# tudelft/CUAHN-VIO

Hardware: AMD Instinct MI355X
Metric: homography preds/sec (frame pairs/s), full 4-block HomographyNet @ 320x224 (higher is better)
Workload: dtype f32 as 2 x fp16 planes (three fp16 MFMAs per product, fp32 accumulate)

## Files before the change

cuahn_vio_amd/csrc/capi_weights.hip:

```cpp
#include "capi_internal.h"

using namespace hnet;

namespace capi {

bool parse_blob(const uint8_t* p, size_t len, Blob& out) {
    if (len < 12 || memcmp(p, "HNETW001", 8) != 0) return false;
    uint32_t n; memcpy(&n, p + 8, 4);
    if (n > 1024) return false;
    size_t pos = 12;
    struct Ent { std::string name; std::vector<uint32_t> dims; uint64_t off; size_t count; };
    std::vector<Ent> ents;
    for (uint32_t i = 0; i < n; i++) {
        if (pos + 4 > len) return false;
        uint32_t ln; memcpy(&ln, p + pos, 4); pos += 4;
        if (ln > 512 || pos + ln + 4 > len) return false;
        Ent e; e.name.assign((const char*)p + pos, ln); pos += ln;
        uint32_t nd; memcpy(&nd, p + pos, 4); pos += 4;
        if (nd > 8 || pos + 4 * nd + 8 > len) return false;
        e.count = 1;
        for (uint32_t d = 0; d < nd; d++) {
            uint32_t v; memcpy(&v, p + pos, 4); pos += 4;
            e.dims.push_back(v);
            if (v != 0 && e.count > (len / 4) / v) return false;
            e.count *= v;
        }
        memcpy(&e.off, p + pos, 8); pos += 8;
        if (e.off % 4) return false;
        ents.push_back(e);
    }
    const size_t data0 = (pos + 63) / 64 * 64;
    if (data0 > len) return false;
    const size_t room = len - data0;
    for (auto& e : ents) {
        if (e.off > room || e.count > (room - (size_t)e.off) / 4) return false;
        out.t.push_back({e.name, Tensor{e.dims, (const float*)(p + data0 + e.off), e.count}});
    }
    return true;
}

template <typename T>
static hipError_t upload(T** dst, const std::vector<T>& v) {
    hipError_t e = dalloc(dst, v.size());
    if (e != hipSuccess) return e;
    return hipMemcpy(*dst, v.data(), v.size() * sizeof(T), hipMemcpyHostToDevice);
}

static std::vector<float> pack_conv(const float* w, const ConvDesc& d, int kp) {
    const int rl = d.ks * d.cin, rlp = kp / d.ks;
    std::vector<float> out((size_t)d.cout * kp, 0.0f);
    for (int co = 0; co < d.cout; co++)
        for (int ci = 0; ci < d.cin; ci++)
            for (int kh = 0; kh < d.ks; kh++)
                for (int kw = 0; kw < d.ks; kw++) {
                    const int r = kw * d.cin + ci;
                    (void)rl;
                    out[(size_t)co * kp + kh * rlp + r] = w[(((size_t)co * d.cin + ci) * d.ks + kh) * d.ks + kw];
                }
    return out;
}

static std::vector<float> pack_first_weights(const float* w, int cout) {
    const int nfrag = cout == 8 ? 28 : 56;
    std::vector<float> out((size_t)nfrag * 64, 0.0f);
    for (int t = 0; t < nfrag; t++)
        for (int l = 0; l < 64; l++) {
            int kh, kk, n;
            if (cout == 8) { kh = t / 4; kk = 4 * (l >> 4) + (t % 4); n = l & 15; }
            else { kh = t / 8; const int q = (t % 8) / 4, e = t % 4; kk = 8 * q + 4 * (l >> 5) + e; n = l & 31; }
            const int kwp = kk >> 1, ci = kk & 1, dx = n / cout, co = n % cout, kw = kwp - dx;
            if (kw >= 0 && kw < 7) out[(size_t)t * 64 + l] = w[(((size_t)co * 2 + ci) * 7 + kh) * 7 + kw];
        }
    return out;
}

static std::vector<float> permute_fc(const float* w, int n_out) {
    std::vector<float> out((size_t)n_out * 5120);
    for (int o = 0; o < n_out; o++)
        for (int c = 0; c < 256; c++)
            for (int pix = 0; pix < 20; pix++) out[(size_t)o * 5120 + pix * 256 + c] = w[(size_t)o * 5120 + c * 20 + pix];
    return out;
}

static inline void wsplit_gemm(float w, int np, uint16_t& a, uint16_t& b, uint16_t& c3) {
    if (np == 2) { split2h(w, a, b); c3 = 0; }
    else split3(w, a, b, c3);
}
int upload_weights(hnet_ctx* c, const Blob& b) {
#define CK(expr)                                                                    \
    do {                                                                            \
        hipError_t e_ = (expr);                                                     \
        if (e_ != hipSuccess) {                                                     \
            fprintf(stderr, "hnet weights: %s: %s\n", #expr, hipGetErrorString(e_)); \
            return HNET_ERR_DEVICE;                                                 \
        }                                                                           \
    } while (0)
    {
        auto fr = [](auto*& p) { if (p) (void)hipFree(p); p = nullptr; };
        for (int l = 0; l < 20; l++) { fr(c->patch_frag[l]); fr(c->conv_w[l]); fr(c->conv_b[l]); fr(c->conv_w16[l]); fr(c->conv_wfrag[l]); fr(c->chain_w[l]); }
        for (int k = 0; k < 3; k++) { fr(c->fc_w[k]); fr(c->fc_b[k]); }
        fr(c->s2_frag[0]); fr(c->s2_frag[3]); fr(c->b30_frag); fr(c->b40_frag); fr(c->b41_frag); fr(c->w1_16); fr(c->b3f_w1); fr(c->b42_w2); fr(c->b42_w3);
        fr(c->w1); fr(c->b1); fr(c->w2); fr(c->b2);
    }
    for (int l = 0; l < 20; l++) {
        const ConvDesc& d = kConvs[l];
        const std::string pre = std::string(d.block == 4 ? "model_last_block_list.0." : "model_part1.") + d.name + ".0.";
        const Tensor* w = b.find(pre + "weight", {(uint32_t)d.cout, (uint32_t)d.cin, (uint32_t)d.ks, (uint32_t)d.ks});
        const Tensor* bi = b.find(pre + "bias", {(uint32_t)d.cout});
        if (!w || !bi) return HNET_ERR_BAD_WEIGHTS;
        if (c->s3 && c->n_planes == 2 && chain_layer(l)) {
            std::vector<uint16_t> fr;
            if (!chain_pack_weights(l, w->data, fr)) return HNET_ERR_BAD_WEIGHTS;
            CK(upload(&c->chain_w[l], fr));
        }
        if (c->s3 && l == 13) {
            std::vector<uint16_t> fr((size_t)5 * 3 * 64 * 8, 0);
            for (int ln = 0; ln < 64; ln++) {
                const int n = ln & 15, gg = ln >> 4, dx = n >> 3, co = n & 7;
                for (int e = 0; e < 4; e++) {
                    const int kk = 4 * gg + e, kw = (kk >> 1) - dx, ci = kk & 1;
                    if (kw < 0 || kw >= 7) continue;
                    uint16_t sp[3];
                    wsplit_np(w->data[(((size_t)co * 2 + ci) * 7 + 6) * 7 + kw], c->n_planes, sp[0], sp[1], sp[2]);
                    for (int pl = 0; pl < 3; pl++) fr[(((size_t)4 * 3 + pl) * 64 + ln) * 8 + e] = sp[pl];
                }
            }
            for (int st = 0; st < 4; st++)
                for (int ln = 0; ln < 64; ln++) {
                    const int n = ln & 15, gg = ln >> 4, kh = 2 * st + (gg >> 1);
                    if (kh >= 7) continue;
                    const int dx = n >> 3, co = n & 7;
                    for (int j = 0; j < 8; j++) {
                        const int kk = 8 * (gg & 1) + j, kw = (kk >> 1) - dx, ci = kk & 1;
                        if (kw < 0 || kw >= 7) continue;
                        uint16_t sp[3];
                        wsplit_np(w->data[(((size_t)co * 2 + ci) * 7 + kh) * 7 + kw], c->n_planes, sp[0], sp[1], sp[2]);
                        for (int pl = 0; pl < 3; pl++) fr[(((size_t)st * 3 + pl) * 64 + ln) * 8 + j] = sp[pl];
                    }
                }
            CK(upload(&c->b40_frag, fr));
        }
        if (c->s3 && l == 7) {
            std::vector<uint16_t> fr((size_t)7 * 3 * 64 * 8, 0);
            for (int kh = 0; kh < 7; kh++)
                for (int ln = 0; ln < 64; ln++) {
                    const int n = ln & 31, hh = ln >> 5, dx = n >> 4, co = n & 15;
                    for (int j = 0; j < 8; j++) {
                        const int kk = 8 * hh + j, kw = (kk >> 1) - dx, ci = kk & 1;
                        if (kw < 0 || kw >= 7) continue;
                        uint16_t sp[3];
                        wsplit_np(w->data[(((size_t)co * 2 + ci) * 7 + kh) * 7 + kw], c->n_planes, sp[0], sp[1], sp[2]);
                        for (int pl = 0; pl < 3; pl++) fr[(((size_t)kh * 3 + pl) * 64 + ln) * 8 + j] = sp[pl];
                    }
                }
            CK(upload(&c->b30_frag, fr));
            c->b30_s3 = true;
        }
        if (c->s3 && l == 8 && c->n_planes == 2) {
            std::vector<uint16_t> f2((size_t)2 * 13 * 2 * 64 * 8, 0);
            for (int nt = 0; nt < 2; nt++)
                for (int st = 0; st < 13; st++)
                    for (int ln = 0; ln < 64; ln++) {
                        const int co = 16 * nt + (ln & 15), gg = ln >> 4, t = 2 * st + (gg >> 1);
                        if (t >= 25) continue;
                        const int kh = t / 5, kw = t % 5;
                        for (int j = 0; j < 8; j++) {
                            const int ci = 8 * (gg & 1) + j;
                            uint16_t a0, a1;
                            split2h(w->data[(((size_t)co * 16 + ci) * 5 + kh) * 5 + kw], a0, a1);
                            f2[((((size_t)nt * 13 + st) * 2 + 0) * 64 + ln) * 8 + j] = a0;
                            f2[((((size_t)nt * 13 + st) * 2 + 1) * 64 + ln) * 8 + j] = a1;
                        }
                    }
            CK(upload(&c->b3f_w1, f2));
        }
        if (c->s3 && (l == 15 || l == 16) && c->n_planes == 2) {
            const int nnt = d.cout / 16, nst = l == 15 ? 5 : 9;
            std::vector<uint16_t> f2((size_t)nnt * nst * 2 * 64 * 8, 0);
            for (int nt = 0; nt < nnt; nt++)
                for (int st = 0; st < nst; st++)
                    for (int ln = 0; ln < 64; ln++) {
                        const int co = 16 * nt + (ln & 15), gg = ln >> 4;
                        const int t = l == 15 ? 2 * st + (gg >> 1) : st;
                        if (t >= 9) continue;
                        const int kh = t / 3, kw = t % 3;
                        for (int j = 0; j < 8; j++) {
                            const int ci = l == 15 ? 8 * (gg & 1) + j : 8 * gg + j;
                            uint16_t a0, a1;
                            split2h(w->data[(((size_t)co * d.cin + ci) * 3 + kh) * 3 + kw], a0, a1);
                            f2[((((size_t)nt * nst + st) * 2 + 0) * 64 + ln) * 8 + j] = a0;
                            f2[((((size_t)nt * nst + st) * 2 + 1) * 64 + ln) * 8 + j] = a1;
                        }
                    }
            CK(upload(l == 15 ? &c->b42_w2 : &c->b42_w3, f2));
        }
        if (c->s3 && conv_is_first_s2(l)) {
            const int nt_n = d.cout / 16;
            std::vector<uint16_t> fr((size_t)nt_n * 4 * 3 * 64 * 8, 0);
            for (int nt = 0; nt < nt_n; nt++)
                for (int st = 0; st < 4; st++)
                    for (int ln = 0; ln < 64; ln++) {
                        const int co = nt * 16 + (ln & 15), gg = ln >> 4, kh = 2 * st + (gg >> 1);
                        if (kh >= 7) continue;
                        for (int j = 0; j < 8; j++) {
                            const int kw = 4 * (gg & 1) + (j >> 1), ci = j & 1;
                            if (kw >= 7) continue;
                            uint16_t sp[3];
                            wsplit_np(w->data[(((size_t)co * 2 + ci) * 7 + kh) * 7 + kw], c->n_planes, sp[0], sp[1], sp[2]);
                            for (int pl = 0; pl < 3; pl++) fr[((((size_t)nt * 4 + st) * 3 + pl) * 64 + ln) * 8 + j] = sp[pl];
                        }
                    }
            CK(upload(&c->s2_frag[l], fr));
            c->first_s2 = true;
        }
        if (c->s3 && conv_is_patch32_layer(l)) {
            std::vector<uint16_t> fr((size_t)4 * 9 * 3 * 64 * 8, 0);
            for (int nt = 0; nt < 4; nt++)
                for (int st = 0; st < 9; st++)
                    for (int ln = 0; ln < 64; ln++) {
                        const int n = nt * 16 + (ln & 15), gg = ln >> 4, kh = st / 3, kw = st % 3;
                        for (int j = 0; j < 8; j++) {
                            const int ci = 8 * gg + j;
                            uint16_t sp[3];
                            wsplit_np(w->data[(((size_t)n * 32 + ci) * 3 + kh) * 3 + kw], c->n_planes, sp[0], sp[1], sp[2]);
                            for (int pl = 0; pl < 3; pl++) fr[((((size_t)nt * 9 + st) * 3 + pl) * 64 + ln) * 8 + j] = sp[pl];
                        }
                    }
            CK(upload(&c->patch_frag[l], fr));
        }
        if (c->s3 && conv_is_patch_layer(l)) {
            const int ks = d.ks, nstep = (ks * ks + 1) / 2;
            std::vector<uint16_t> fr((size_t)2 * nstep * 3 * 64 * 8, 0);
            for (int nt = 0; nt < 2; nt++)
                for (int st = 0; st < nstep; st++)
                    for (int ln = 0; ln < 64; ln++) {
                        const int n = nt * 16 + (ln & 15), gg = ln >> 4, t = 2 * st + (gg >> 1);
                        if (t >= ks * ks) continue;
                        const int kh = t / ks, kw = t % ks;
                        for (int j = 0; j < 8; j++) {
                            const int ci = 8 * (gg & 1) + (((gg & 1) && !c->patch_b128) ? (j + 4) % 8 : j);
                            uint16_t sp[3];
                            wsplit_np(w->data[(((size_t)n * 16 + ci) * ks + kh) * ks + kw], c->n_planes, sp[0], sp[1], sp[2]);
                            for (int pl = 0; pl < 3; pl++) fr[((((size_t)nt * nstep + st) * 3 + pl) * 64 + ln) * 8 + j] = sp[pl];
                        }
                    }
            CK(upload(&c->patch_frag[l], fr));
        }
        if (conv_is_first_direct(l)) CK(upload(&c->conv_w[l], pack_first_weights(w->data, d.cout)));
        else {
            const std::vector<float> packed = pack_conv(w->data, d, conv_padded_k(l));
            CK(upload(&c->conv_w[l], packed));
            if (c->s3 && l == 14) {
                std::vector<uint16_t> fr((size_t)7 * 3 * 64 * 8, 0);
                for (int st = 0; st < 7; st++)
                    for (int ln = 0; ln < 64; ln++) {
                        const int n = ln & 15, gg = ln >> 4, t = c->n_planes == 2 ? b41_tap(st, gg) : 4 * st + gg;
                        if (t < 0 || t >= 25) continue;
                        const int kh = t / 5, kw = t % 5;
                        for (int j = 0; j < 8; j++) {
                            const int ci = (c->n_planes != 2 && (gg & 1)) ? (j + 4) % 8 : j;
                            uint16_t sp[3];
                            wsplit_np(w->data[(((size_t)n * 8 + ci) * 5 + kh) * 5 + kw], c->n_planes, sp[0], sp[1], sp[2]);
                            for (int pl = 0; pl < 3; pl++) fr[(((size_t)st * 3 + pl) * 64 + ln) * 8 + j] = sp[pl];
                        }
                    }
                CK(upload(&c->b41_frag, fr));
            }
            if (c->s3 && conv_is_s3_layer(l)) {
                std::vector<uint16_t> pl(packed.size() * 3);
                for (size_t i = 0; i < packed.size(); i++)
                    wsplit_gemm(packed[i], c->n_planes, pl[i], pl[packed.size() + i], pl[2 * packed.size() + i]);
                CK(upload(&c->conv_w16[l], pl));
            }
            if (c->n_planes == 2 && conv_region_layer(l)) {
                const int ntap = d.ks * d.ks, ntap_pad = conv_region_taps_padded(l), nchunk = d.cin / 64;
                std::vector<uint16_t> fr((size_t)(d.cout / 16) * nchunk * ntap_pad * 2 * 2 * 64 * 8, 0);
                for (int nt = 0; nt < d.cout / 16; nt++)
                    for (int cc = 0; cc < nchunk; cc++)
                        for (int t = 0; t < ntap; t++)
                            for (int st = 0; st < 2; st++)
                                for (int ln = 0; ln < 64; ln++)
                                    for (int e = 0; e < 8; e++) {
                                        const int n = nt * 16 + (ln & 15), ci = 64 * cc + 32 * st + 8 * (ln >> 4) + e;
                                        uint16_t sp[3];
                                        wsplit_gemm(w->data[(((size_t)n * d.cin + ci) * d.ks + t / d.ks) * d.ks + t % d.ks], 2, sp[0], sp[1], sp[2]);
                                        const size_t base = ((((size_t)(nt * nchunk + cc) * ntap_pad + t) * 2 + st) * 2) * 64 * 8;
                                        fr[base + (size_t)ln * 8 + e] = sp[0];
                                        fr[base + 64 * 8 + (size_t)ln * 8 + e] = sp[1];
                                    }
                CK(upload(&c->conv_wfrag[l], fr));
            }
        }
        CK(upload(&c->conv_b[l], std::vector<float>(bi->data, bi->data + d.cout)));
    }
    for (int k = 0; k < 3; k++) {
        const std::string pre = "model_part1.fc_block_" + std::to_string(k + 1) + ".";
        const Tensor* w = b.find(pre + "weight", {8, 5120});
        const Tensor* bi = b.find(pre + "bias", {8});
        if (!w || !bi) return HNET_ERR_BAD_WEIGHTS;
        CK(upload(&c->fc_w[k], permute_fc(w->data, 8)));
        CK(upload(&c->fc_b[k], std::vector<float>(bi->data, bi->data + 8)));
    }
    {
        static const char* heads[2] = {"fc_block_4_mean", "fc_block_4_uncertainty"};
        std::vector<float> w1, b1, w2, b2;
        for (int h = 0; h < 2; h++) {
            const std::string pre = std::string("model_last_block_list.0.") + heads[h] + ".";
            const Tensor* tw1 = b.find(pre + "1.weight", {256, 5120});
            const Tensor* tb1 = b.find(pre + "1.bias", {256});
            const Tensor* tw2 = b.find(pre + "4.weight", {8, 256});
            const Tensor* tb2 = b.find(pre + "4.bias", {8});
            if (!tw1 || !tb1 || !tw2 || !tb2) return HNET_ERR_BAD_WEIGHTS;
            std::vector<float> p = permute_fc(tw1->data, 256);
            w1.insert(w1.end(), p.begin(), p.end());
            b1.insert(b1.end(), tb1->data, tb1->data + 256);
            w2.insert(w2.end(), tw2->data, tw2->data + 8 * 256);
            b2.insert(b2.end(), tb2->data, tb2->data + 8);
        }
        CK(upload(&c->w1, w1)); CK(upload(&c->b1, b1)); CK(upload(&c->w2, w2)); CK(upload(&c->b2, b2));
        c->w1_feat_scale = 1.0f;
        if (c->s3) {
            int e = 0;
            if (c->n_planes == 2) {
                float m = 0.f;
                for (float v : w1) m = std::max(m, std::fabs(v));
                if (m > 0.f && m < 0x1p-15f) e = std::min(-7 - std::ilogb(m), 24);
            }
            const float up = std::ldexp(1.0f, e);
            c->w1_feat_scale = std::ldexp(1.0f, -e);
            std::vector<uint16_t> pl(w1.size() * 3);
            for (size_t i = 0; i < w1.size(); i++) wsplit_gemm(w1[i] * up, c->n_planes, pl[i], pl[w1.size() + i], pl[2 * w1.size() + i]);
            CK(upload(&c->w1_16, pl));
        }
    }

    return HNET_OK;
#undef CK
}

}
```

cuahn_vio_amd/csrc/igemm_region.h:

```cpp
#pragma once
#include "igemm_pipe.h"

namespace hnet {

template <int CIN_, int KS_, int P_, int RP_, bool KSPLIT_, int HI_, int WI_>
struct RegionCfg {
    static constexpr int CIN = CIN_, KS = KS_, P = P_, RP = RP_, PAD = (KS_ - 1) / 2;
    static constexpr int HI = HI_, WI = WI_, HO = (HI_ + 1) / 2, WO = WI_ / 2;
    static_assert(WI_ % 2 == 0, "the parity images assume an even input width");
    static constexpr bool KSPLIT = KSPLIT_;
    static constexpr int TM = 5, BM = 80, BN = KSPLIT_ ? 64 : 128, NWAVE = 8, NT = 512;
    static constexpr int NCHUNK = CIN / 64, NTAP = KS * KS;
    static constexpr int TAPS_X = KSPLIT_ ? (NTAP + 1) / 2 : NTAP;
    static constexpr int NTAP_PAD = KSPLIT_ ? 2 * TAPS_X : NTAP;
    static constexpr int DEPTH = 5;
    static_assert((2 * TAPS_X) % DEPTH == 0, "weight-fragment ring");
    static constexpr int REG_PLANE = (RP + 16) * 64;
    static constexpr int REG_BUF = 2 * REG_PLANE;
    static constexpr int LDS_BYTES = 2 * REG_BUF * 2;
    static constexpr int RG = RP / 8;
    static_assert(RP % 8 == 0 && LDS_BYTES <= 160 * 1024 && CIN % 64 == 0, "region");
    static constexpr size_t wfrag_halves(int n) { return (size_t)(n / 16) * NCHUNK * NTAP_PAD * 2 * 2 * 64 * 8; }
};

template <class C, bool OUT32>
__global__ __launch_bounds__(512, 2) void igemm_s3_region_kernel(S3Params p) {
    constexpr int TM = C::TM, BN = C::BN, NWAVE = C::NWAVE, CIN = C::CIN, KS = C::KS, PAD = C::PAD;
    constexpr int REG_PLANE = C::REG_PLANE, REG_BUF = C::REG_BUF, NTAP = C::NTAP, NCHUNK = C::NCHUNK;
    constexpr int DEPTH = C::DEPTH, NTAP_PAD = C::NTAP_PAD;
    extern __shared__ __attribute__((aligned(16))) uint16_t smem_r[];

    const int tid = threadIdx.x, lane = tid & 63;
    const int wave = __builtin_amdgcn_readfirstlane(tid >> 6);
    const int khalf = C::KSPLIT ? wave >> 2 : 0, wn = C::KSPLIT ? wave & 3 : wave;
    constexpr int R = C::HO * C::WO, HW = C::HI * C::WI;
    const int rows_tile = C::P * R;
    int mt, n0;
    {
        const int nx = gridDim.x, ny = gridDim.y, total = nx * ny;
        const int lin = blockIdx.x + blockIdx.y * nx;
        const int xcd = lin & 7, idx = lin >> 3;
        const int base = total >> 3, rem = total & 7;
        const int Lt = xcd * base + min(xcd, rem) + idx;
        mt = Lt / ny;
        n0 = (Lt % ny) * BN;
    }
    const int m0 = mt * rows_tile, pair0 = mt * C::P;
    const int m_end = min(p.M, m0 + rows_tile);
    const int px_total = (p.M / R) * HW;

    const __amdgpu_buffer_rsrc_t rA = __builtin_amdgcn_make_buffer_rsrc((void*)p.A, 0, 0x7FFFFFF0, 0x00020000);
    const __amdgpu_buffer_rsrc_t rW = __builtin_amdgcn_make_buffer_rsrc((void*)p.Wp, 0, 0x7FFFFFF0, 0x00020000);
    const int a_pl = (int)(p.a_plane * 2);

    {
        const u32x4 z = {0u, 0u, 0u, 0u};
        *reinterpret_cast<u32x4*>(&smem_r[(tid >> 8) * REG_BUF + ((tid >> 7) & 1) * REG_PLANE + C::RP * 64 + (tid & 127) * 8]) = z;
    }

    const int grow = lane >> 3, gphys = lane & 7;
    constexpr int RGW = (C::RG + NWAVE - 1) / NWAVE;
    constexpr int Wo = C::WO, hh_e = (C::HI + 1) >> 1, hh_o = C::HI >> 1;
    constexpr int ps_e = (hh_e * Wo + 1) & ~1, ps_o = (hh_o * Wo + 1) & ~1;
    constexpr int base2 = 2 * C::P * ps_e;
    uint32_t rvoff[RGW];
#pragma unroll
    for (int j = 0; j < RGW; j++) {
        const int q = (wave + NWAVE * j) * 8 + grow;
        const int yo = q >= base2, qq = yo ? q - base2 : q, ps = yo ? ps_o : ps_e, hh = yo ? hh_o : hh_e;
        const int xo = qq >= C::P * ps, q3 = xo ? qq - C::P * ps : qq;
        const int pl_ = yo ? q3 / ps_o : q3 / ps_e;
        const int t = q3 - pl_ * ps, Y = t / Wo, xh = t - Y * Wo;
        const int T = pl_ * R + t;
        const int gq = (pair0 + pl_) * HW + (2 * Y + yo) * C::WI + 2 * xh + xo;
        const bool ok = q < base2 + 2 * C::P * ps_o && t < hh * Wo && gq < px_total;
        rvoff[j] = ok ? (uint32_t)((gq * CIN + (gphys ^ (2 * ((T >> 1) & 3))) * 8) * 2) : S3_OOB;
    }
    auto dma_region = [&](int c) {
#pragma unroll
        for (int j = 0; j < RGW; j++) {
            const int g = wave + NWAVE * j;
            if (g < C::RG) {
                const uint32_t vo = rvoff[j];
#pragma unroll
                for (int pl = 0; pl < 2; pl++) {
                    const int so = c * 128 + pl * a_pl;
                    __builtin_amdgcn_raw_ptr_buffer_load_lds(rA, (lds_ptr_t)(smem_r + (c & 1) * REG_BUF + pl * REG_PLANE + g * 512), 16, vo, so, 0, 0);
                }
            }
        }
    };

    const uint32_t wlane = (uint32_t)(lane * 16);
    const int wtile0 = ((n0 >> 4) + wn) * (NCHUNK * NTAP_PAD);
    const int t_lo_w = khalf * C::TAPS_X;
    bf16x8 fw[DEPTH][2];
    auto load_w = [&](int slot, int c, int sidx) {
#if defined(HNET_REGION_ABLATE) && HNET_REGION_ABLATE == 1
        if (c | (sidx >= DEPTH)) return;
#endif
        const int so = (wtile0 + c * NTAP_PAD + t_lo_w) * 4096 + sidx * 2048;
#pragma unroll
        for (int pl = 0; pl < 2; pl++) {
            const int so2 = so + pl * 1024;
            fw[slot][pl] = __builtin_bit_cast(bf16x8, __builtin_amdgcn_raw_buffer_load_b128(rW, wlane, so2, 0));
        }
    };

    const int r16 = lane & 15, g16 = lane >> 4;
    int qe_b[TM], qo_b[TM], tt0[TM];
    uint32_t okb[TM];
#pragma unroll
    for (int i = 0; i < TM; i++) {
        const int ml = i * 16 + r16;
        const bool ok = m0 + ml < m_end;
        const int pl_ = ml / R, rem = ml - pl_ * R, oy = rem / Wo, ox = rem - oy * Wo;
        const int t0 = oy * Wo + ox;
        qe_b[i] = (pl_ * ps_e + t0) * 128;
        qo_b[i] = (base2 + pl_ * ps_o + t0) * 128;
        tt0[i] = pl_ * R + t0;
        uint32_t bits = 0;
#pragma unroll
        for (int k = 0; k < KS; k++) {
            bits |= ((unsigned)(2 * oy - PAD + k) < (unsigned)C::HI) ? (1u << k) : 0u;
            bits |= ((unsigned)(2 * ox - PAD + k) < (unsigned)C::WI) ? (1u << (8 + k)) : 0u;
        }
        okb[i] = ok ? bits : 0u;
    }
    bf16x8 fa[2][TM][2];
    int a_byte[TM];
    constexpr int xoff_e = C::P * ps_e * 128, xoff_o = C::P * ps_o * 128;
    auto tap_addr = [&](int t) {
#if defined(HNET_REGION_ABLATE) && HNET_REGION_ABLATE == 2
        if (t != t_lo_w) return;
#endif
        const int kh = t / KS, kw = t - kh * KS;
        const int ey = kh - PAD, ex = kw - PAD;
        const int yo = ey & 1, xo = ex & 1, dt = (ey >> 1) * Wo + (ex >> 1);
        const int s_b = (xo ? (yo ? xoff_o : xoff_e) : 0) + dt * 128;
        const uint32_t need = t < NTAP ? ((1u << kh) | (1u << (8 + kw))) : 0xFFFFFFFFu;
#pragma unroll
        for (int i = 0; i < TM; i++) {
            int t0_ = tt0[i], qs_ = yo ? qo_b[i] : qe_b[i];
            asm volatile("" : "+v"(t0_), "+v"(qs_));
            const int T = t0_ + dt;
            const bool ok = (okb[i] & need) == need;
            const int qb = ok ? qs_ + s_b : (C::RP + (T & 15)) * 128;
            a_byte[i] = qb | ((g16 ^ (T & 6)) << 4);
        }
    };
    auto read_a = [&](int set, int buf, int st) {
#if defined(HNET_REGION_ABLATE) && HNET_REGION_ABLATE == 4
        if (buf | st) return;
#endif
        const unsigned char* rg = reinterpret_cast<const unsigned char*>(smem_r + buf * REG_BUF);
#pragma unroll
        for (int i = 0; i < TM; i++)
#pragma unroll
            for (int pl = 0; pl < 2; pl++)
                fa[set][i][pl] = *reinterpret_cast<const bf16x8*>(rg + pl * (REG_PLANE * 2) + (a_byte[i] ^ (st << 6)));
    };

    f32x4_m16 acc[TM], accl[TM];
#pragma unroll
    for (int i = 0; i < TM; i++) { acc[i] = f32x4_m16{0.f, 0.f, 0.f, 0.f}; accl[i] = f32x4_m16{0.f, 0.f, 0.f, 0.f}; }
    auto mfma = [&](int set, int slot) {
#if defined(HNET_REGION_ABLATE) && HNET_REGION_ABLATE == 3
        {
#pragma unroll
            for (int i = 0; i < TM; i++) asm volatile("" ::"v"(fa[set][i][0]), "v"(fa[set][i][1]));
            asm volatile("" ::"v"(fw[slot][0]), "v"(fw[slot][1]));
            return;
        }
#endif
#pragma unroll
        for (int i = 0; i < TM; i++) {
            bf16x8 w3[3] = {fw[slot][0], fw[slot][1], fw[slot][0]}, a3[3] = {fa[set][i][0], fa[set][i][1], fa[set][i][0]};
            s3_mfma16_2acc(acc[i], accl[i], w3, a3);
        }
    };

    constexpr int NJ = C::TAPS_X, NS = 2 * NJ;
    const int t_lo = t_lo_w;

    dma_region(0);
    if (NCHUNK > 1) dma_region(1);
#pragma unroll
    for (int d = 0; d < DEPTH; d++) load_w(d, 0, d);
    __builtin_amdgcn_s_waitcnt(0x0070);
    __builtin_amdgcn_s_barrier();
    __builtin_amdgcn_sched_barrier(0);

    for (int c = 0; c < NCHUNK; c++) {
        const int buf = c & 1;
        tap_addr(t_lo);
        read_a(0, buf, 0);
#pragma unroll
        for (int j = 0; j < NJ; j++) {
            read_a(1, buf, 1);
            mfma(0, (2 * j) % DEPTH);
            __builtin_amdgcn_sched_barrier(0);
            if (2 * j + DEPTH < NS) load_w((2 * j) % DEPTH, c, 2 * j + DEPTH);
            else if (c + 1 < NCHUNK) load_w((2 * j) % DEPTH, c + 1, 2 * j + DEPTH - NS);
            if (j + 1 < NJ) {
                tap_addr(t_lo + j + 1);
                read_a(0, buf, 0);
            }
            mfma(1, (2 * j + 1) % DEPTH);
            __builtin_amdgcn_sched_barrier(0);
            if (2 * j + 1 + DEPTH < NS) load_w((2 * j + 1) % DEPTH, c, 2 * j + 1 + DEPTH);
            else if (c + 1 < NCHUNK) load_w((2 * j + 1) % DEPTH, c + 1, 2 * j + 1 + DEPTH - NS);
        }
        if (c + 1 < NCHUNK) {
            static_assert(DEPTH == 5, "s_waitcnt immediate: vmcnt(10) lgkmcnt(0)");
            __builtin_amdgcn_s_waitcnt(0x007A);
            __builtin_amdgcn_s_barrier();
            __builtin_amdgcn_sched_barrier(0);
            if (c + 2 < NCHUNK) dma_region(c + 2);
        }
    }

#pragma unroll
    for (int i = 0; i < TM; i++) acc[i] += accl[i] * S3_F16_INV;

    if constexpr (C::KSPLIT) {
        __builtin_amdgcn_s_waitcnt(0xc07f);
        __builtin_amdgcn_s_barrier();
        float* red = reinterpret_cast<float*>(smem_r);
        if (khalf) {
#pragma unroll
            for (int i = 0; i < TM; i++) *reinterpret_cast<f32x4_m16*>(&red[(wn * TM + i) * 256 + lane * 4]) = acc[i];
        }
        __syncthreads();
        if (khalf) return;
#pragma unroll
        for (int i = 0; i < TM; i++) acc[i] += *reinterpret_cast<const f32x4_m16*>(&red[(wn * TM + i) * 256 + lane * 4]);
    }

    const int em = lane & 15, eg = lane >> 4;
    const int n = n0 + wn * 16 + 4 * eg;
    const f32x4_m16 bv = *reinterpret_cast<const f32x4_m16*>(p.bias + n);
#pragma unroll
    for (int i = 0; i < TM; i++) {
        const int m = m0 + i * 16 + em;
        f32x4_m16 v = acc[i];
        {
            const s3p::f32x2_p x0 = s3p::f32x2_p{v[0], v[1]} + s3p::f32x2_p{bv[0], bv[1]}, x1 = s3p::f32x2_p{v[2], v[3]} + s3p::f32x2_p{bv[2], bv[3]};
            const s3p::f32x2_p t0 = x0 * 0.1f, t1 = x1 * 0.1f;
            v[0] = s3p::vmax1(x0[0], t0[0]); v[1] = s3p::vmax1(x0[1], t0[1]); v[2] = s3p::vmax1(x1[0], t1[0]); v[3] = s3p::vmax1(x1[1], t1[1]);
        }
        if (m < m_end) {
            if constexpr (OUT32) {
                *reinterpret_cast<f32x4_m16*>(p.out32 + (size_t)m * p.N + n) = v;
            } else {
                uint32_t pa[3], pb[3];
                s3p::split_pair<2>(v[0], v[1], pa);
                s3p::split_pair<2>(v[2], v[3], pb);
#pragma unroll
                for (int pl = 0; pl < 2; pl++)
                    *reinterpret_cast<uint2*>(p.out16 + pl * p.o_plane + (size_t)m * p.N + n) = make_uint2(pa[pl], pb[pl]);
            }
        }
    }
}

}
```

cuahn_vio_amd/csrc/kernels.h:

```cpp
#pragma once
#include <hip/hip_runtime.h>
#include <stdint.h>

namespace hnet {

struct ConvDesc {
    const char* name;
    int cin, cout, ks, stride;
    int seg;
    int block;
};
extern const ConvDesc kConvs[20];
int conv_padded_k(int layer);
bool conv_is_first_direct(int layer);
inline int conv_out_dim(int n, int ks, int stride) { return (n + 2 * ((ks - 1) / 2) - ks) / stride + 1; }

hipError_t launch_conv(int layer, const float* in, int batch, int h, int w, const float* wpacked,
                       const float* bias, float* out, hipStream_t s, float* ws = nullptr, size_t ws_floats = 0,
                       uint16_t* out16 = nullptr, size_t o_plane = 0);

bool conv_is_s3_layer(int layer);
bool conv_region_layer(int layer);
int conv_region_taps_padded(int layer);
constexpr int SPLITK_TICKETS = 4096;
struct LatIO {
    uint32_t* tickets;
    int kernels;
    bool heads_one_launch;
    bool mask_ready;
};
bool heads_fc1_one_launch(int batch, int n_local, int n_planes);
hipError_t launch_conv_s3(int layer, const uint16_t* in, size_t in_plane, int batch, int h, int w, const uint16_t* wplanes,
                          size_t w_plane, const float* bias, uint16_t* out16, size_t o_plane, float* out32, hipStream_t s,
                          float* ws = nullptr, size_t ws_floats = 0, const uint16_t* wfrag = nullptr, int n_planes = 3, int tile = 0, LatIO* lat = nullptr);
bool conv_is_patch_layer(int layer);
bool conv_is_patch32_layer(int layer);
hipError_t launch_conv_patch(int layer, const uint16_t* in, size_t i_plane, int batch, int h, int w, const void* wfrag,
                             const float* bias, uint16_t* out16, size_t o_plane, hipStream_t s, int n_planes = 3,
                             bool b128 = false ,
                             int rb5 = 1 );
hipError_t launch_conv_first_s3(const float* x_in, const void* wfrag, const float* bias, uint16_t* out16, size_t o_plane, int batch,
                                int h, int w, hipStream_t s, int n_planes = 3);
inline bool conv_is_first_s2(int layer) { return layer == 0 || layer == 3; }
hipError_t launch_conv_first_s2(int layer, const float* x_in, const void* wfrag, const float* bias, uint16_t* out16, size_t o_plane, int batch,
                                hipStream_t s, int n_planes = 3);
struct B4Warp { const uint8_t* img1; const uint8_t* img2; const float* H; };
inline bool block4_warp_in_supported(const void* img1, const void* img2, int pix_fmt_is_u8, int n_planes) {
    return pix_fmt_is_u8 && n_planes == 2 && ((((uintptr_t)img1 | (uintptr_t)img2) & 3) == 0);
}
hipError_t launch_block4_fused(const void* x_in, size_t x_plane, const void* w0frag, const float* bias0, const void* w1frag, const float* bias1,
                               uint16_t* out16, size_t o_plane, int batch, hipStream_t s, int flags = 0 , int n_planes = 3,
                               const B4Warp* warp = nullptr);
hipError_t launch_block3_fused(const float* x_in, const void* w0frag, const float* bias0, const void* w1frag, const float* bias1, uint16_t* out16,
                               size_t o_plane, int batch, hipStream_t s, int n_planes);
hipError_t launch_block42_fused(const uint16_t* in16, size_t i_plane, const void* w2frag, const float* bias2, const void* w3frag, const float* bias3,
                                uint16_t* out16, size_t o_plane, int batch, hipStream_t s, int n_planes);
hipError_t conv_kernels_init_device();
hipError_t launch_heads_fc1_s3(const float* feat, int batch, int n_local, int s_begin, float p, uint64_t mc_seed,
                               uint64_t pair_seq0, const uint16_t* w1planes, const float* b1, float* hidden,
                               uint16_t* feat16, size_t f_plane, uint8_t* mask, hipStream_t s,
                               float* ws = nullptr, size_t ws_floats = 0, const uint64_t* seq_dev = nullptr, int n_planes = 3, int tile = 0,
                               LatIO* lat = nullptr ,
                               const uint64_t* seq_tab = nullptr ,
                               float feat_scale = 1.0f );
hipError_t launch_nchw_f32_to_nhwc_s3(const float* in, uint16_t* out, size_t o_plane, int batch, int c, int h, int w, hipStream_t s, int n_planes = 3);
hipError_t launch_nhwc_s3_to_nchw_f32(const uint16_t* in, size_t i_plane, float* out, int batch, int c, int h, int w, hipStream_t s, int n_planes = 3);

hipError_t launch_heads_fc1(const float* feat, int batch, int n_local, int s_begin, float p, uint64_t mc_seed,
                            uint64_t pair_seq0, const float* w1packed, const float* b1, float* hidden, hipStream_t s,
                            float* ws = nullptr, size_t ws_floats = 0, const uint64_t* seq_dev = nullptr, const uint64_t* seq_tab = nullptr);

constexpr int B4_PADX = 5, B4_PADY = 5, B4_WP = 336, B4_HP = 235;
constexpr int B42_PADX = 3, B42_PADY = 3, B42_WP = 164, B42_HP = 115;
constexpr size_t B42_IMG = (size_t)B42_HP * B42_WP;
hipError_t launch_s3_repitch(const uint16_t* src, size_t src_plane, uint16_t* dst, size_t dst_plane, int batch, int h, int w, int c, int hp, int wp, int pady,
                             int padx, bool to_padded, hipStream_t s, int n_planes);
constexpr int b41_tap(int st, int g) {
    if (st < 5) return g * 5 + st;
    if (st == 5) return g == 0 ? 20 : g == 2 ? 21 : -1;
    return g == 0 ? 22 : g == 2 ? 23 : g == 3 ? 24 : -1;
}

hipError_t launch_prep(const void* img1, const void* img2, int pix_fmt, const float* H, int k, float* out,
                       int batch, hipStream_t s, uint32_t* out_s3 = nullptr, size_t s3_plane = 0, int n_planes = 3, bool exact = true);
struct FcArgs {
    const float* feat;
    const float* wfc;
    const float* bfc;
    const float* H_in;
    const float* prior;
    float* H_out;
    uint8_t* mask;
    int mask_blocks, n_local, s_begin;
    uint32_t thr;
    uint64_t mc_seed, pair_seq0;
    const uint64_t* seq_dev;
    const uint64_t* seq_tab;
    const float* fc_part;
};
bool prep_fc_supported(const void* img1, const void* img2, int k, bool has_out_s3);
hipError_t launch_prep_fc(const void* img1, const void* img2, int pix_fmt, const FcArgs& fc, int k, float* out, int batch, hipStream_t s,
                          uint32_t* out_s3, size_t s3_plane, int n_planes, bool exact);
hipError_t launch_f32_nhwc_to_s3pad(const float* x, uint32_t* out, size_t s3_plane, int batch, int n_planes, hipStream_t s);
hipError_t launch_s3pad_to_f32_nhwc(const uint32_t* in, size_t s3_plane, float* x, int batch, int n_planes, hipStream_t s);

hipError_t launch_undistort(const uint8_t* raw, int rows, int cols, int stride, const float* map_x, const float* map_y, uint8_t* out,
                            hipStream_t s);
hipError_t launch_session_scatter(const uint8_t* staged, const int32_t* dst_slot, int n, int n_slots, uint8_t* ring, hipStream_t s);
hipError_t launch_session_gather(const uint8_t* ring, int n_slots, const int32_t* pair_slot, int n, uint8_t* prev, uint8_t* curr, hipStream_t s);
hipError_t launch_session_remap(const uint8_t* raw, size_t raw_frame, int rows, int cols, const int32_t* dst_slot, const int32_t* cam, const float* const* maps,
                                int n_cams, int n, int n_slots, uint8_t* ring, hipStream_t s);
hipError_t launch_errmap(const void* img1, const void* img2, int pix_fmt, const float* H, float* out,
                         uint8_t* out_u8, int batch, hipStream_t s);

hipError_t launch_warp_f32(const float* img, const float* H, float* out, int batch, hipStream_t s);

hipError_t launch_prior_dlt(const float* prior, float* H, int batch, hipStream_t s);
hipError_t launch_dlt(const float* dst, float* H, int n, hipStream_t s);

hipError_t launch_block_fc_dlt(const float* feat, const float* wfc, const float* bfc, const float* H_in,
                               float* H_out, int batch, hipStream_t s);

hipError_t launch_heads_fc2(const float* hidden, int batch, int n_local, int s_begin, float p, uint64_t mc_seed,
                            uint64_t pair_seq0, const float* w2, const float* b2, float* mean_s, float* logvar_s,
                            hipStream_t s, const uint64_t* seq_dev = nullptr, uint32_t* flag = nullptr ,
                            const uint64_t* seq_tab = nullptr);

hipError_t launch_mc_finish(const float* mean_s, const float* logvar_s, int n, const float* H1, int batch,
                            float* mean, float* cov, float* Htot, hipStream_t s, uint32_t* flag = nullptr,
                            int mean_stride = 8, int cov_stride = 64 ,
                            int n_local = 0, size_t rank_stride = 0 );

constexpr int HEADS_FC2_FINISH_MAX_N = 64;
hipError_t launch_heads_fc2_finish(const float* hidden, int batch, int n_local, int s_begin, float p, uint64_t mc_seed, uint64_t pair_seq0, const float* w2,
                                   const float* b2, const float* H1, float* mean, float* cov, float* Htot, hipStream_t s,
                                   const uint64_t* seq_dev = nullptr, uint32_t* flag = nullptr, int mean_stride = 8, int cov_stride = 64,
                                   const uint64_t* seq_tab = nullptr);

hipError_t launch_nchw_to_nhwc(const float* in, float* out, int batch, int c, int h, int w, hipStream_t s);
hipError_t launch_nhwc_to_nchw(const float* in, float* out, int batch, int c, int h, int w, hipStream_t s);

}
```

cuahn_vio_amd/csrc/kernels_conv.hip:

```cpp
#include "s3_dispatch.h"

namespace hnet {

const ConvDesc kConvs[20] = {
    {"block_1_1", 2, 128, 7, 2, 16, 1}, {"block_1_2", 128, 128, 5, 2, 32, 1}, {"block_1_3", 128, 256, 3, 2, 32, 1},
    {"block_2_1", 2, 64, 7, 2, 16, 2},  {"block_2_2", 64, 128, 5, 2, 32, 2},  {"block_2_3", 128, 256, 3, 2, 32, 2},
    {"block_2_4", 256, 256, 3, 2, 32, 2},
    {"block_3_0", 2, 16, 7, 1, 16, 3},  {"block_3_1", 16, 32, 5, 2, 16, 3},   {"block_3_2", 32, 64, 3, 2, 32, 3},
    {"block_3_3", 64, 128, 3, 2, 32, 3}, {"block_3_4", 128, 256, 3, 2, 32, 3}, {"block_3_5", 256, 256, 3, 2, 32, 3},
    {"block_4_0", 2, 8, 7, 1, 16, 4},   {"block_4_1", 8, 16, 5, 2, 8, 4},     {"block_4_2", 16, 32, 3, 2, 16, 4},
    {"block_4_3", 32, 64, 3, 2, 32, 4}, {"block_4_4", 64, 128, 3, 2, 32, 4},  {"block_4_5", 128, 256, 3, 2, 32, 4},
    {"block_4_6", 256, 256, 3, 2, 32, 4},
};

bool conv_is_first_direct(int layer) { return layer == 7 || layer == 13; }

int conv_padded_k(int layer) {
    const ConvDesc& d = kConvs[layer];
    if (conv_is_first_direct(layer)) return 0;
    const int rl = d.ks * d.cin;
    const int spr = (rl + d.seg - 1) / d.seg;
    return d.ks * spr * d.seg;
}

int splitk_min_iters(long tiles) { return tiles < 16 ? 4 : 3; }
int splitk_target_blocks(long tiles) { return tiles < 16 ? 192 : 384; }

template <class L, int BM, int BN, int WGM, int MF>
static hipError_t run(IgemmParams p, hipStream_t s, float* ws, size_t ws_floats) {
    dim3 grid((p.M + BM - 1) / BM, (p.N + BN - 1) / BN, 1);
    const long tiles = (long)grid.x * grid.y;
    const int n_iter = (p.Kp + IG_BK - 1) / IG_BK;
    int split = 1;
    if (ws && tiles < 192 && n_iter >= 8 && (p.N % 4) == 0) {
        split = (int)std::min<long>(std::min<long>(n_iter / splitk_min_iters(tiles), (splitk_target_blocks(tiles) + tiles - 1) / tiles), 64);
        const size_t per = (size_t)p.M * p.N;
        if ((size_t)split * per > ws_floats) split = (int)(ws_floats / per);
        if (split < 2) split = 1;
    }
    p.k_split = split;
    p.partial = ws;
    grid.z = split;

    hipLaunchKernelGGL((igemm_kernel<L, BM, BN, WGM, MF>), grid, dim3(256), 0, s, p);
    if (split > 1) {
        const size_t total4 = (size_t)p.M * p.N / 4;
        hipLaunchKernelGGL(splitk_reduce_kernel, dim3((unsigned)((total4 + 255) / 256)), dim3(256), 0, s, ws, split, p.M, p.N, p.bias, p.out);
    }
    return hipGetLastError();
}

template <int CIN, int KS, int STRIDE, int SEG, int COUT>
static hipError_t run_conv(const IgemmParams& p, hipStream_t s, float* ws, size_t wsn) {
    typedef ConvLoader<CIN, KS, STRIDE, SEG> L;
    if constexpr (COUT <= 16) {
        return run<L, 128, 16, 4, 16>(p, s, ws, wsn);
    } else if constexpr (COUT == 32) {
        return run<L, 128, 32, 4, 32>(p, s, ws, wsn);
    } else {
        return run<L, 64, 64, 2, 32>(p, s, ws, wsn);
    }
}

hipError_t launch_conv(int layer, const float* in, int batch, int h, int w, const float* wpacked,
                       const float* bias, float* out, hipStream_t s, float* ws, size_t wsn, uint16_t* out16, size_t o_plane) {
    if (layer < 0 || layer >= 20) return hipErrorInvalidValue;
    const ConvDesc& d = kConvs[layer];
    IgemmParams p = {};
    p.A = in; p.Wp = wpacked; p.bias = bias; p.out = out;
    p.out16 = out16; p.o_plane = o_plane;
    if (out16) { ws = nullptr; wsn = 0; }
    p.H = h; p.W = w;
    p.Ho = conv_out_dim(h, d.ks, d.stride);
    p.Wo = conv_out_dim(w, d.ks, d.stride);
    p.M = batch * p.Ho * p.Wo;
    p.N = d.cout;
    p.Kp = conv_padded_k(layer);
    if (conv_is_first_direct(layer)) {
        if (d.cout == 8) {
            const int tx = (w + 63) / 64, ty = (h + 15) / 16;
            hipLaunchKernelGGL(conv7_c2_s1_kernel<8>, dim3((unsigned)(batch * tx * ty)), dim3(256), 0, s, in, wpacked, bias, out, out16, o_plane, h, w, tx, ty);
        } else {
            const int tx = (w + 31) / 32, ty = (h + 15) / 16;
            hipLaunchKernelGGL(conv7_c2_s1_kernel<16>, dim3((unsigned)(batch * tx * ty)), dim3(256), 0, s, in, wpacked, bias, out, out16, o_plane, h, w, tx, ty);
        }
        return hipGetLastError();
    }
    switch (layer) {
        case 0:  return run_conv<2, 7, 2, 16, 128>(p, s, ws, wsn);
        case 1:  return run_conv<128, 5, 2, 32, 128>(p, s, ws, wsn);
        case 2: case 5: case 11: case 18: return run_conv<128, 3, 2, 32, 256>(p, s, ws, wsn);
        case 3:  return run_conv<2, 7, 2, 16, 64>(p, s, ws, wsn);
        case 4:  return run_conv<64, 5, 2, 32, 128>(p, s, ws, wsn);
        case 6: case 12: case 19: return run_conv<256, 3, 2, 32, 256>(p, s, ws, wsn);
        case 8:  return run_conv<16, 5, 2, 16, 32>(p, s, ws, wsn);
        case 9: case 16: return run_conv<32, 3, 2, 32, 64>(p, s, ws, wsn);
        case 10: case 17: return run_conv<64, 3, 2, 32, 128>(p, s, ws, wsn);
        case 14: return run_conv<8, 5, 2, 8, 16>(p, s, ws, wsn);
        case 15: return run_conv<16, 3, 2, 16, 32>(p, s, ws, wsn);
    }
    return hipErrorInvalidValue;
}

HNET_S3_DISPATCH_INSTANCES(, 3)
HNET_S3_DISPATCH_INSTANCES(extern, 1)
HNET_S3_DISPATCH_INSTANCES(extern, 2)

bool conv_is_s3_layer(int layer) { return kConvs[layer].cin >= 8; }
bool conv_region_layer(int layer) { return layer == 1 || layer == 2 || layer == 6 || layer == 12 || layer == 19; }
int conv_region_taps_padded(int layer) { return layer == 1 ? 25 : 10; }
bool conv_is_patch_layer(int layer) { return layer == 8 || layer == 15; }
bool conv_is_patch32_layer(int layer) { return layer == 9 || layer == 16; }

hipError_t conv_kernels_init_device() {
    hipError_t e = conv_kernels_init_device_np<3>();
    if (e == hipSuccess) e = conv_kernels_init_device_np<1>();
    return e != hipSuccess ? e : conv_kernels_init_device_np<2>();
}

#define HNET_NP(fn, ...) (n_planes == 1 ? fn<1>(__VA_ARGS__) : n_planes == 2 ? fn<2>(__VA_ARGS__) : fn<3>(__VA_ARGS__))

hipError_t launch_block4_fused(const void* x_in, size_t x_plane, const void* w0frag, const float* bias0, const void* w1frag, const float* bias1,
                               uint16_t* out16, size_t o_plane, int batch, hipStream_t s, int flags, int n_planes, const B4Warp* warp) {
    return HNET_NP(launch_block4_fused_np, x_in, x_plane, w0frag, bias0, w1frag, bias1, out16, o_plane, batch, s, flags, warp);
}

hipError_t launch_block42_fused(const uint16_t* in16, size_t i_plane, const void* w2frag, const float* bias2, const void* w3frag, const float* bias3,
                                uint16_t* out16, size_t o_plane, int batch, hipStream_t s, int n_planes) {
    return HNET_NP(launch_block42_fused_np, in16, i_plane, w2frag, bias2, w3frag, bias3, out16, o_plane, batch, s);
}

hipError_t launch_block3_fused(const float* x_in, const void* w0frag, const float* bias0, const void* w1frag, const float* bias1, uint16_t* out16,
                               size_t o_plane, int batch, hipStream_t s, int n_planes) {
    return HNET_NP(launch_block3_fused_np, x_in, w0frag, bias0, w1frag, bias1, out16, o_plane, batch, s);
}

hipError_t launch_conv_first_s3(const float* x_in, const void* wfrag, const float* bias, uint16_t* out16, size_t o_plane, int batch,
                                int h, int w, hipStream_t s, int n_planes) {
    return HNET_NP(launch_conv_first_s3_np, x_in, wfrag, bias, out16, o_plane, batch, h, w, s);
}

hipError_t launch_conv_first_s2(int layer, const float* x_in, const void* wfrag, const float* bias, uint16_t* out16, size_t o_plane, int batch,
                                hipStream_t s, int n_planes) {
    return HNET_NP(launch_conv_first_s2_np, layer, x_in, wfrag, bias, out16, o_plane, batch, s);
}

hipError_t launch_conv_patch(int layer, const uint16_t* in, size_t i_plane, int batch, int h, int w, const void* wfrag,
                             const float* bias, uint16_t* out16, size_t o_plane, hipStream_t s, int n_planes, bool b128, int rb5) {
    return HNET_NP(launch_conv_patch_np, layer, in, i_plane, batch, h, w, wfrag, bias, out16, o_plane, s, b128, rb5);
}

hipError_t launch_heads_fc1_s3(const float* feat, int batch, int n_local, int s_begin, float p_drop, uint64_t mc_seed,
                               uint64_t pair_seq0, const uint16_t* w1planes, const float* b1, float* hidden,
                               uint16_t* feat16, size_t f_plane, uint8_t* mask, hipStream_t s, float* ws, size_t wsn,
                               const uint64_t* seq_dev, int n_planes, int tile, LatIO* lat, const uint64_t* seq_tab, float feat_scale) {
    return HNET_NP(launch_heads_fc1_s3_np, feat, batch, n_local, s_begin, p_drop, mc_seed, pair_seq0, w1planes, b1, hidden, feat16, f_plane, mask, s, ws, wsn, seq_dev, tile, lat,
                   seq_tab, feat_scale);
}

bool heads_fc1_one_launch(int batch, int n_local, int n_planes) { return n_planes == 2 && batch <= 8 && n_local <= 16 * HL_MAXG; }

hipError_t launch_conv_s3(int layer, const uint16_t* in, size_t in_plane, int batch, int h, int w, const uint16_t* wplanes,
                          size_t w_plane, const float* bias, uint16_t* out16, size_t o_plane, float* out32, hipStream_t s,
                          float* ws, size_t wsn, const uint16_t* wfrag, int n_planes, int tile, LatIO* lat) {
    return HNET_NP(launch_conv_s3_np, layer, in, in_plane, batch, h, w, wplanes, w_plane, bias, out16, o_plane, out32, s, ws, wsn, wfrag, tile, lat);
}

__global__ void s3_repitch_kernel(const uint16_t* __restrict__ src, size_t src_plane, uint16_t* __restrict__ dst, size_t dst_plane, int batch, int h, int w, int cch,
                                  int hp, int wp, int pady, int padx, int to_padded, int n_planes) {
    const long n = (long)n_planes * batch * h * w * cch;
    const long i = (long)blockIdx.x * blockDim.x + threadIdx.x;
    if (i >= n) return;
    const int ch = (int)(i % cch);
    long r = i / cch;
    const int x = (int)(r % w); r /= w;
    const int y = (int)(r % h); r /= h;
    const int b = (int)(r % batch);
    const int pl = (int)(r / batch);
    const size_t plain = (size_t)pl * (to_padded ? src_plane : dst_plane) + ((((size_t)b * h + y) * w + x) * cch + ch) * 8;
    const size_t padded = (size_t)pl * (to_padded ? dst_plane : src_plane) + ((((size_t)b * hp + y + pady) * wp + x + padx) * cch + ch) * 8;
    if (to_padded) *reinterpret_cast<u32x4*>(dst + padded) = *reinterpret_cast<const u32x4*>(src + plain);
    else *reinterpret_cast<u32x4*>(dst + plain) = *reinterpret_cast<const u32x4*>(src + padded);
}
hipError_t launch_s3_repitch(const uint16_t* src, size_t src_plane, uint16_t* dst, size_t dst_plane, int batch, int h, int w, int c, int hp, int wp, int pady,
                             int padx, bool to_padded, hipStream_t s, int n_planes) {
    if (c % 8) return hipErrorInvalidValue;
    const long n = (long)n_planes * batch * h * w * (c / 8);
    hipLaunchKernelGGL(s3_repitch_kernel, dim3((unsigned)((n + 255) / 256)), dim3(256), 0, s, src, src_plane, dst, dst_plane, batch, h, w, c / 8, hp, wp, pady, padx,
                       to_padded ? 1 : 0, n_planes);
    return hipGetLastError();
}

hipError_t launch_nchw_f32_to_nhwc_s3(const float* in, uint16_t* out, size_t o_plane, int batch, int c, int h, int w, hipStream_t s, int n_planes) {
    const long n = (long)batch * c * h * w;
    hipLaunchKernelGGL(nchw_f32_to_nhwc_s3_kernel, dim3((unsigned)((n + 255) / 256)), dim3(256), 0, s, in, out, o_plane, batch, c, h * w, n_planes);
    return hipGetLastError();
}
hipError_t launch_nhwc_s3_to_nchw_f32(const uint16_t* in, size_t i_plane, float* out, int batch, int c, int h, int w, hipStream_t s, int n_planes) {
    const long n = (long)batch * c * h * w;
    hipLaunchKernelGGL(nhwc_s3_to_nchw_f32_kernel, dim3((unsigned)((n + 255) / 256)), dim3(256), 0, s, in, i_plane, out, batch, c, h * w, n_planes);
    return hipGetLastError();
}

hipError_t launch_heads_fc1(const float* feat, int batch, int n_local, int s_begin, float p_drop, uint64_t mc_seed,
                            uint64_t pair_seq0, const float* w1packed, const float* b1, float* hidden, hipStream_t s,
                            float* ws, size_t wsn, const uint64_t* seq_dev, const uint64_t* seq_tab) {
    IgemmParams p = {};
    p.A = feat; p.Wp = w1packed; p.bias = b1; p.out = hidden;
    p.M = batch * n_local;
    p.N = 512;
    p.Kp = 5120;
    p.n_local = n_local;
    p.s_begin = s_begin;
    p.thr = hnet_drop_threshold(p_drop);
    p.scale = 1.0f / (1.0f - p_drop);
    p.mc_seed = mc_seed;
    p.pair_seq0 = pair_seq0;
    p.seq_dev = seq_dev;
    p.seq_tab = seq_tab;
    return run<HeadLoader, 64, 64, 2, 32>(p, s, ws, wsn);
}

}
```

Baseline: 210,600.

## Split region-kernel K across halves by tap-half steps to drop padded tap

Reindexes the region implicit-GEMM K loop in units of half-tap steps (two 32-channel steps per tap) so the two K-split wave halves each get exactly half the steps, instead of padding the 3x3 tap count from 9 to 10. This removes the dummy padded tap's MFMAs and weight fragment loads. The weight fragment packing drops the padding, and the weight ring depth is reduced to 3 for the K-split case, with the waitcnt immediate derived from the depth. The loop is templated on the half index, which raises code size, and the shallower ring may hide less load latency.

```diff
diff --git a/cuahn_vio_amd/csrc/capi_weights.hip b/cuahn_vio_amd/csrc/capi_weights.hip
--- a/cuahn_vio_amd/csrc/capi_weights.hip
+++ b/cuahn_vio_amd/csrc/capi_weights.hip
@@ -273,8 +273,8 @@
                 CK(upload(&c->conv_w16[l], pl));
             }
             if (c->n_planes == 2 && conv_region_layer(l)) {
-                const int ntap = d.ks * d.ks, ntap_pad = conv_region_taps_padded(l), nchunk = d.cin / 64;
-                std::vector<uint16_t> fr((size_t)(d.cout / 16) * nchunk * ntap_pad * 2 * 2 * 64 * 8, 0);
+                const int ntap = d.ks * d.ks, nstep = 2 * ntap, nchunk = d.cin / 64;
+                std::vector<uint16_t> fr((size_t)(d.cout / 16) * nchunk * nstep * 2 * 64 * 8, 0);
                 for (int nt = 0; nt < d.cout / 16; nt++)
                     for (int cc = 0; cc < nchunk; cc++)
                         for (int t = 0; t < ntap; t++)
@@ -284,7 +284,7 @@
                                         const int n = nt * 16 + (ln & 15), ci = 64 * cc + 32 * st + 8 * (ln >> 4) + e;
                                         uint16_t sp[3];
                                         wsplit_gemm(w->data[(((size_t)n * d.cin + ci) * d.ks + t / d.ks) * d.ks + t % d.ks], 2, sp[0], sp[1], sp[2]);
-                                        const size_t base = ((((size_t)(nt * nchunk + cc) * ntap_pad + t) * 2 + st) * 2) * 64 * 8;
+                                        const size_t base = (((size_t)(nt * nchunk + cc) * nstep + 2 * t + st) * 2) * 64 * 8;
                                         fr[base + (size_t)ln * 8 + e] = sp[0];
                                         fr[base + 64 * 8 + (size_t)ln * 8 + e] = sp[1];
                                     }
diff --git a/cuahn_vio_amd/csrc/igemm_region.h b/cuahn_vio_amd/csrc/igemm_region.h
--- a/cuahn_vio_amd/csrc/igemm_region.h
+++ b/cuahn_vio_amd/csrc/igemm_region.h
@@ -1,4 +1,5 @@
 #pragma once
+#include <type_traits>
 #include "igemm_pipe.h"
 
 namespace hnet {
@@ -11,23 +12,23 @@
     static constexpr bool KSPLIT = KSPLIT_;
     static constexpr int TM = 5, BM = 80, BN = KSPLIT_ ? 64 : 128, NWAVE = 8, NT = 512;
     static constexpr int NCHUNK = CIN / 64, NTAP = KS * KS;
-    static constexpr int TAPS_X = KSPLIT_ ? (NTAP + 1) / 2 : NTAP;
-    static constexpr int NTAP_PAD = KSPLIT_ ? 2 * TAPS_X : NTAP;
-    static constexpr int DEPTH = 5;
-    static_assert((2 * TAPS_X) % DEPTH == 0, "weight-fragment ring");
+    static constexpr int NSTEP = 2 * NTAP;
+    static constexpr int NS = KSPLIT_ ? NSTEP / 2 : NSTEP;
+    static constexpr int DEPTH = KSPLIT_ ? 3 : 5;
+    static_assert(NS % DEPTH == 0 && 2 * DEPTH <= 15, "weight-fragment ring (vmcnt(2 DEPTH) is a four-bit immediate below)");
     static constexpr int REG_PLANE = (RP + 16) * 64;
     static constexpr int REG_BUF = 2 * REG_PLANE;
     static constexpr int LDS_BYTES = 2 * REG_BUF * 2;
     static constexpr int RG = RP / 8;
     static_assert(RP % 8 == 0 && LDS_BYTES <= 160 * 1024 && CIN % 64 == 0, "region");
-    static constexpr size_t wfrag_halves(int n) { return (size_t)(n / 16) * NCHUNK * NTAP_PAD * 2 * 2 * 64 * 8; }
+    static constexpr size_t wfrag_halves(int n) { return (size_t)(n / 16) * NCHUNK * NSTEP * 2 * 64 * 8; }
 };
 
 template <class C, bool OUT32>
 __global__ __launch_bounds__(512, 2) void igemm_s3_region_kernel(S3Params p) {
     constexpr int TM = C::TM, BN = C::BN, NWAVE = C::NWAVE, CIN = C::CIN, KS = C::KS, PAD = C::PAD;
-    constexpr int REG_PLANE = C::REG_PLANE, REG_BUF = C::REG_BUF, NTAP = C::NTAP, NCHUNK = C::NCHUNK;
-    constexpr int DEPTH = C::DEPTH, NTAP_PAD = C::NTAP_PAD;
+    constexpr int REG_PLANE = C::REG_PLANE, REG_BUF = C::REG_BUF, NCHUNK = C::NCHUNK;
+    constexpr int DEPTH = C::DEPTH, NSTEP = C::NSTEP, NS = C::NS;
     extern __shared__ __attribute__((aligned(16))) uint16_t smem_r[];
 
     const int tid = threadIdx.x, lane = tid & 63;
@@ -92,14 +93,13 @@
     };
 
     const uint32_t wlane = (uint32_t)(lane * 16);
-    const int wtile0 = ((n0 >> 4) + wn) * (NCHUNK * NTAP_PAD);
-    const int t_lo_w = khalf * C::TAPS_X;
+    const int wstep0 = ((n0 >> 4) + wn) * (NCHUNK * NSTEP) + khalf * NS;
     bf16x8 fw[DEPTH][2];
     auto load_w = [&](int slot, int c, int sidx) {
 #if defined(HNET_REGION_ABLATE) && HNET_REGION_ABLATE == 1
         if (c | (sidx >= DEPTH)) return;
 #endif
-        const int so = (wtile0 + c * NTAP_PAD + t_lo_w) * 4096 + sidx * 2048;
+        const int so = (wstep0 + c * NSTEP + sidx) * 2048;
 #pragma unroll
         for (int pl = 0; pl < 2; pl++) {
             const int so2 = so + pl * 1024;
@@ -130,15 +130,15 @@
     bf16x8 fa[2][TM][2];
     int a_byte[TM];
     constexpr int xoff_e = C::P * ps_e * 128, xoff_o = C::P * ps_o * 128;
-    auto tap_addr = [&](int t) {
+    auto tap_addr = [&](int t, bool first) {
 #if defined(HNET_REGION_ABLATE) && HNET_REGION_ABLATE == 2
-        if (t != t_lo_w) return;
+        if (!first) return;
 #endif
         const int kh = t / KS, kw = t - kh * KS;
         const int ey = kh - PAD, ex = kw - PAD;
         const int yo = ey & 1, xo = ex & 1, dt = (ey >> 1) * Wo + (ex >> 1);
         const int s_b = (xo ? (yo ? xoff_o : xoff_e) : 0) + dt * 128;
-        const uint32_t need = t < NTAP ? ((1u << kh) | (1u << (8 + kw))) : 0xFFFFFFFFu;
+        const uint32_t need = (1u << kh) | (1u << (8 + kw));
 #pragma unroll
         for (int i = 0; i < TM; i++) {
             int t0_ = tt0[i], qs_ = yo ? qo_b[i] : qe_b[i];
@@ -180,9 +180,6 @@
         }
     };
 
-    constexpr int NJ = C::TAPS_X, NS = 2 * NJ;
-    const int t_lo = t_lo_w;
-
     dma_region(0);
     if (NCHUNK > 1) dma_region(1);
 #pragma unroll
@@ -191,34 +188,35 @@
     __builtin_amdgcn_s_barrier();
     __builtin_amdgcn_sched_barrier(0);
 
-    for (int c = 0; c < NCHUNK; c++) {
-        const int buf = c & 1;
-        tap_addr(t_lo);
-        read_a(0, buf, 0);
-#pragma unroll
-        for (int j = 0; j < NJ; j++) {
-            read_a(1, buf, 1);
-            mfma(0, (2 * j) % DEPTH);
-            __builtin_amdgcn_sched_barrier(0);
-            if (2 * j + DEPTH < NS) load_w((2 * j) % DEPTH, c, 2 * j + DEPTH);
-            else if (c + 1 < NCHUNK) load_w((2 * j) % DEPTH, c + 1, 2 * j + DEPTH - NS);
-            if (j + 1 < NJ) {
-                tap_addr(t_lo + j + 1);
-                read_a(0, buf, 0);
-            }
-            mfma(1, (2 * j + 1) % DEPTH);
-            __builtin_amdgcn_sched_barrier(0);
-            if (2 * j + 1 + DEPTH < NS) load_w((2 * j + 1) % DEPTH, c, 2 * j + 1 + DEPTH);
-            else if (c + 1 < NCHUNK) load_w((2 * j + 1) % DEPTH, c + 1, 2 * j + 1 + DEPTH - NS);
-        }
-        if (c + 1 < NCHUNK) {
-            static_assert(DEPTH == 5, "s_waitcnt immediate: vmcnt(10) lgkmcnt(0)");
-            __builtin_amdgcn_s_waitcnt(0x007A);
-            __builtin_amdgcn_s_barrier();
-            __builtin_amdgcn_sched_barrier(0);
-            if (c + 2 < NCHUNK) dma_region(c + 2);
-        }
-    }
+    auto k_loop = [&](auto KH) {
+        constexpr int S0 = decltype(KH)::value * NS;
+        for (int c = 0; c < NCHUNK; c++) {
+            const int buf = c & 1;
+            tap_addr(S0 >> 1, true);
+            read_a(0, buf, S0 & 1);
+#pragma unroll
+            for (int i = 0; i < NS; i++) {
+                if (i + 1 < NS) {
+                    if (((S0 + i + 1) & 1) == 0) tap_addr((S0 + i + 1) >> 1, false);
+                    read_a((i + 1) & 1, buf, (S0 + i + 1) & 1);
+                }
+                mfma(i & 1, i % DEPTH);
+                __builtin_amdgcn_sched_barrier(0);
+                if (i + DEPTH < NS) load_w(i % DEPTH, c, i + DEPTH);
+                else if (c + 1 < NCHUNK) load_w(i % DEPTH, c + 1, i + DEPTH - NS);
+            }
+            if (c + 1 < NCHUNK) {
+                __builtin_amdgcn_s_waitcnt(0x0070 | (2 * DEPTH));
+                __builtin_amdgcn_s_barrier();
+                __builtin_amdgcn_sched_barrier(0);
+                if (c + 2 < NCHUNK) dma_region(c + 2);
+            }
+        }
+    };
+    if constexpr (C::KSPLIT) {
+        if (khalf) k_loop(std::integral_constant<int, 1>{});
+        else k_loop(std::integral_constant<int, 0>{});
+    } else k_loop(std::integral_constant<int, 0>{});
 
 #pragma unroll
     for (int i = 0; i < TM; i++) acc[i] += accl[i] * S3_F16_INV;
diff --git a/cuahn_vio_amd/csrc/kernels.h b/cuahn_vio_amd/csrc/kernels.h
--- a/cuahn_vio_amd/csrc/kernels.h
+++ b/cuahn_vio_amd/csrc/kernels.h
@@ -21,7 +21,6 @@
 
 bool conv_is_s3_layer(int layer);
 bool conv_region_layer(int layer);
-int conv_region_taps_padded(int layer);
 constexpr int SPLITK_TICKETS = 4096;
 struct LatIO {
     uint32_t* tickets;
diff --git a/cuahn_vio_amd/csrc/kernels_conv.hip b/cuahn_vio_amd/csrc/kernels_conv.hip
--- a/cuahn_vio_amd/csrc/kernels_conv.hip
+++ b/cuahn_vio_amd/csrc/kernels_conv.hip
@@ -108,7 +108,6 @@
 
 bool conv_is_s3_layer(int layer) { return kConvs[layer].cin >= 8; }
 bool conv_region_layer(int layer) { return layer == 1 || layer == 2 || layer == 6 || layer == 12 || layer == 19; }
-int conv_region_taps_padded(int layer) { return layer == 1 ? 25 : 10; }
 bool conv_is_patch_layer(int layer) { return layer == 8 || layer == 15; }
 bool conv_is_patch32_layer(int layer) { return layer == 9 || layer == 16; }
 
```

Result: no change. 211,100, median of 6 (+0.3%).
